# KarypisLab/SLIM

Measured on AMD Instinct MI355X. Metric: item-columns solved/sec (whole node), higher is better.
Workload: dtype f32

## Files before the change

slim_amd/csrc/cd_tile.hpp:

```cpp
#pragma once
#include <type_traits>

#include "cd_wave.hpp"

namespace slimamd {

#ifndef SLIM_TILE_END_ALIGNED
#define SLIM_TILE_END_ALIGNED 1
#endif

constexpr int kTileNW = 16;
constexpr int kTileKMax = 32;
constexpr float kInactive = -__builtin_huge_valf();
__device__ __forceinline__ bool tile_active(float xv) { return xv > -3.0e38f; }

__device__ __forceinline__ void pin(float& v) { asm volatile("" : "+v"(v)); }
__device__ __forceinline__ void pin(int& v) { asm volatile("" : "+v"(v)); }

template <int N>
__device__ __forceinline__ int row_bcast_c(int v) {
  return __builtin_amdgcn_update_dpp(0, v, 0x150 + N, 0xF, 0xF, true);
}
__device__ __forceinline__ int row_bcast(int v, int n) {
  switch (n & 15) {
    case 0: return row_bcast_c<0>(v);
    case 1: return row_bcast_c<1>(v);
    case 2: return row_bcast_c<2>(v);
    case 3: return row_bcast_c<3>(v);
    case 4: return row_bcast_c<4>(v);
    case 5: return row_bcast_c<5>(v);
    case 6: return row_bcast_c<6>(v);
    case 7: return row_bcast_c<7>(v);
    case 8: return row_bcast_c<8>(v);
    case 9: return row_bcast_c<9>(v);
    case 10: return row_bcast_c<10>(v);
    case 11: return row_bcast_c<11>(v);
    case 12: return row_bcast_c<12>(v);
    case 13: return row_bcast_c<13>(v);
    case 14: return row_bcast_c<14>(v);
    default: return row_bcast_c<15>(v);
  }
}
__device__ __forceinline__ float row_bcast(float v, int n) {
  return __int_as_float(row_bcast(__float_as_int(v), n));
}

template <class T>
__device__ __forceinline__ T ld_off(const void* base, const uint32_t byte_off) {
  return *reinterpret_cast<const T*>(reinterpret_cast<const char*>(base) + byte_off);
}

typedef unsigned long long tile_gran_t;

__device__ __forceinline__ void gran_store(tile_gran_t* p, uint32_t epoch, float v) {
  __hip_atomic_store(p, ((tile_gran_t)epoch << 32) | (tile_gran_t)__float_as_uint(v),
                     __ATOMIC_RELAXED, __HIP_MEMORY_SCOPE_AGENT);
}
__device__ __forceinline__ tile_gran_t gran_load(const tile_gran_t* p) {
  return __hip_atomic_load(p, __ATOMIC_RELAXED, __HIP_MEMORY_SCOPE_AGENT);
}

__device__ __forceinline__ int tile_block_id(const SolveArgs& S) {
  const int b = (int)blockIdx.x, g = (int)gridDim.x;
  return S.xcd_swizzle ? (b & 7) * (g >> 3) + (b >> 3) : b;
}

struct GramStore {
  float* G;
  int64_t G_ld;
  const int32_t* gram_pos;
  const float* atypart;
  int64_t x_stride;
  int32_t gram_part16, gram_accum, gram_store;
};
template <int P, int NW>
__device__ __noinline__ void gram_store_lines(const GramStore S, const int* s_item, const int cid, const int mk,
                                              const int K_, const int base, const int ncols, const int wave,
                                              const int lane) {
  const int K = uni(K_);
  float* const G = reinterpret_cast<float*>(uni(reinterpret_cast<int64_t>(S.G)));
  const int64_t G_ld = uni(S.G_ld), x_stride = uni(S.x_stride);
  const float* const part0 =
      reinterpret_cast<const float*>(uni(reinterpret_cast<int64_t>(S.atypart))) + (int64_t)uni(cid) * K * x_stride;
  const bool p16 = uni(S.gram_part16) != 0, accum = uni(S.gram_accum) != 0, mirror = uni(S.gram_store) == 1;
  const int nblk = (uni(ncols) + 63) >> 6;
  const int per = (nblk + K - 1) / K;
  const int bend = (uni(mk) + 1) * per < nblk ? (uni(mk) + 1) * per : nblk;
  for (int blk = uni(mk) * per + uni(wave); blk < bend; blk += NW) {
    const int i = blk * 64 + lane;
    const int pi = i < ncols ? S.gram_pos[i] : -1;
    const bool keep = pi >= base;
    if (__ballot(keep) == 0ull) continue;
    if (!keep) continue;
    for (int h = 0; h < P / 8; ++h) {
      float a[8];
      if (p16) {
        uint32_t n[8];
#pragma unroll
        for (int e = 0; e < 8; ++e) n[e] = 0u;
        const uint4* src = reinterpret_cast<const uint4*>(reinterpret_cast<const uint16_t*>(part0) + (int64_t)i * P) + h;
#pragma unroll 4
        for (int k = 0; k < K; ++k) {
          const uint4 v = *src;
          src = reinterpret_cast<const uint4*>(reinterpret_cast<const float*>(src) + x_stride);
          n[0] += v.x & 0xFFFFu;
          n[1] += v.x >> 16;
          n[2] += v.y & 0xFFFFu;
          n[3] += v.y >> 16;
          n[4] += v.z & 0xFFFFu;
          n[5] += v.z >> 16;
          n[6] += v.w & 0xFFFFu;
          n[7] += v.w >> 16;
        }
#pragma unroll
        for (int e = 0; e < 8; ++e) a[e] = (float)n[e];
      } else {
#pragma unroll
        for (int e = 0; e < 8; ++e) a[e] = 0.0f;
        const float4* src = reinterpret_cast<const float4*>(part0 + (int64_t)i * P) + 2 * h;
#pragma unroll 2
        for (int k = 0; k < K; ++k) {
          const float4 v = src[0], w = src[1];
          src = reinterpret_cast<const float4*>(reinterpret_cast<const float*>(src) + x_stride);
          a[0] += v.x;
          a[1] += v.y;
          a[2] += v.z;
          a[3] += v.w;
          a[4] += w.x;
          a[5] += w.y;
          a[6] += w.z;
          a[7] += w.w;
        }
      }
      int it[8];
#pragma unroll
      for (int e = 0; e < 8; ++e) it[e] = uni(s_item[8 * h + e]);
      if (accum) {
#pragma unroll
        for (int e = 0; e < 8; ++e)
          if (it[e] >= 0) a[e] += G[(int64_t)it[e] * G_ld + i];
      }
#pragma unroll
      for (int e = 0; e < 8; ++e) {
        if (it[e] >= 0) {
          G[(int64_t)it[e] * G_ld + i] = a[e];
// ... 473 lines not shown
          sim = S.simtype == 0 ? a / cn_i : (S.simtype == 1 ? a / ((cn_i + s_cn[qq]) - a) : a);
        }
        x[idx] = sim;
      }
      auto keyof = [](const float f) -> uint32_t {
        const uint32_t b = __float_as_uint(f);
        return (b & 0x80000000u) ? ~b : (b | 0x80000000u);
      };
      const uint32_t key_ninf = keyof(kInactive);
      for (int pass = 0; pass < 4; ++pass) {
        const int shift = 24 - 8 * pass;
        for (int k = tid; k < P * 256; k += NT) hist[k] = 0u;
        __syncthreads();
        for (int64_t idx = tid; idx < n; idx += NT) {
          const int qq = (int)(idx & (P - 1));
          const uint32_t key = keyof(x[idx]);
          if (key == key_ninf) continue;
          const uint32_t hi_mask = pass == 0 ? 0u : (0xFFFFFFFFu << (shift + 8));
          if ((key & hi_mask) == s_prefix[qq]) atomicAdd(&hist[qq * 256 + ((key >> shift) & 255u)], 1u);
        }
        __syncthreads();
        if (tid < P) {
          uint32_t want = s_want[tid], d = 255u;
          for (;; --d) {
            const uint32_t c = hist[tid * 256 + d];
            if (c >= want || d == 0u) break;
            want -= c;
          }
          s_prefix[tid] |= d << shift;
          s_want[tid] = want;
        }
        __syncthreads();
      }
#pragma unroll
      for (int pp = 0; pp < PPW; ++pp) {
        const int pq = wave + pp * NW;
        const uint32_t T = s_prefix[pq];
        int quota = (int)s_want[pq], na = 0;
        for (int ib = 0; ib < ncols; ib += 64) {
          const int i = ib + lane;
          const uint32_t key = i < ncols ? keyof(x[(int64_t)i * P + pq]) : key_ninf;
          const bool cand = key != key_ninf;
          const bool tie = cand && key == T;
          const uint64_t mt = __ballot(tie);
          const bool act = cand && (key > T || (tie && __popcll(mt & lane_lt) < quota));
          quota -= __popcll(mt) < quota ? __popcll(mt) : quota;
          if (i < ncols) x[(int64_t)i * P + pq] = act ? 0.0f : kInactive;
          na += __popcll(__ballot(act));
        }
        if (lane == 0) s_na[pq] = na;
      }
    } else if (S.gram_mode == 3 && S.gram_store != 0) {
      const GramStore gs{S.G, S.G_ld, S.gram_pos, S.atypart, S.x_stride, S.gram_part16, S.gram_accum, S.gram_store};
      gram_store_lines<P, NW>(gs, s_item, cid, mk, K, base, ncols, wave, lane);
    } else if (S.gram_mode == 3) {
      const int64_t n = (int64_t)ncols * P;
      const int64_t per = (n + K - 1) / K;
      const int64_t hi = (mk + 1) * per < n ? (mk + 1) * per : n;
      for (int64_t idx = mk * per + tid; idx < hi; idx += NT) {
        const int i = (int)(idx >> LOGP), qq = (int)(idx & (P - 1));
        const int it = s_item[qq];
        const int pi = S.gram_pos[i];
        if (pi >= base && it >= 0) {
          float a = 0.0f;
          if (S.gram_part16) {
            uint32_t n = 0u;
            for (int k = 0; k < K; ++k)
              n += reinterpret_cast<const uint16_t*>(S.atypart + (int64_t)(cid * K + k) * S.x_stride)[idx];
            a = (float)n;
          } else {
            for (int k = 0; k < K; ++k) a += S.atypart[(int64_t)(cid * K + k) * S.x_stride + idx];
          }
          if (S.gram_accum) a += S.G[(int64_t)it * S.G_ld + i];
          S.G[(int64_t)it * S.G_ld + i] = a;
          if (pi >= base + P) S.G[(int64_t)i * S.G_ld + it] = a;
        }
      }
    } else {
      const int64_t n = (int64_t)ncols * P;
      for (int64_t idx = tid; idx < n; idx += NT) {
        const int i = (int)(idx >> LOGP), qq = (int)(idx & (P - 1));
        const int it = s_item[qq];
        float a = 0.0f;
        if (cached) {
          a = gram_t[idx];
        } else {
          for (int k = 0; k < K; ++k)
            a += S.atypart[(int64_t)(cid * K + k) * S.x_stride + idx];
          if (gram_t != nullptr && mk == 0) gram_t[idx] = a;
        }
        const bool act = it >= 0 && i != it && a > l1;
        x[idx] = act ? 0.0f : kInactive;
        if (act) atomicAdd(&s_na[qq], 1);
      }
    }
    __syncthreads();
    if (S.gram_mode == 3) continue;

    const bool warm = FOLD != 0 && S.icolptr != nullptr && !FSLIM;
    if (warm) {
#pragma unroll
      for (int pp = 0; pp < PPW; ++pp) {
        const int pq = wave + pp * NW;
        const int witem = s_item[pq];
        if (witem >= 0 && witem < S.incols) {
          const int64_t ws = uni(S.icolptr[witem]), we = uni(S.icolptr[witem + 1]);
          for (int64_t e = ws + lane; e < we; e += 64) {
// ... 592 lines not shown
```

slim_amd/csrc/cd_wave.hpp:

```cpp
#pragma once
#include <hip/hip_runtime.h>

#include <cstdint>

#include "cd_perm.hpp"

namespace slimamd {

struct DevMatrix {
  int32_t nrows, ncols;
  int64_t nnz;
  const int64_t* rowptr;
  const int32_t* rowind;
  const float* rowval;
  const int64_t* colptr;
  const int32_t* colind;
  const float* colval;
  const float* cnorm;
  const float* csq;
};

struct SolveArgs {
  float l1, l2, opt_tol;
  int32_t maxniters;
  uint32_t seed;
  int32_t nnbrs;
  int32_t simtype;
  const int32_t* order;
  int32_t nwork;
  int32_t* queue;
  const int64_t* icolptr;
  const int32_t* icolind;
  const float* icolval;
  int32_t incols;
  float* slab;
  int64_t slab_stride;
  int32_t nrows_pad, ncols_pad;
  float* xslab;
  int64_t x_stride;
  int32_t* ulist;
  int64_t u_stride;
  int32_t ngroups;
  uint64_t* trace;
  int32_t cluster;
  const int32_t* ubounds;
  const int64_t* csplit;
  unsigned long long* mailbox;
  float* atypart;
  int32_t exact_gram;
  int32_t bm_shift, bm_words;
  int32_t nheavy;
  int32_t cluster_hi;
  const int32_t* ubounds_hi;
  const int64_t* csplit_hi;
  unsigned long long* mailbox_hi;
  int32_t* queue_hi;
  int64_t nnz_last;
  int32_t hi_prefetch;
  int32_t shard_count, shard_index;
  int32_t xcd_swizzle;
  float* gram;
  int32_t gram_mode;
  float* G;
  int64_t G_ld;
  int32_t* tile_nunion;
  const int32_t* gram_pos;
  int32_t gram_bits;
  int32_t gram_split_stride;
  int32_t gram_accum;
  const uint4* gview;
  const int64_t* gview_base;
  const uint16_t* gview_cnt;
  int32_t gview_ngroups;
  int32_t gview_range0;
  int32_t gview_sentinel;
  int32_t gram_part16;
  int32_t gram_store;
  float* g_save;
  const float* g_load;
  int64_t g_stride;
  int32_t* out_cnt;
  int64_t* out_off;
  int32_t* out_ind;
  float* out_val;
  unsigned long long* out_cursor;
  int64_t out_cap;
  int32_t* overflow;
  int32_t* st_na;
  int32_t* st_sweeps;
  int32_t* st_conv;
  int64_t* st_G;
  int64_t* st_D;
  int64_t* st_U;
  int64_t* st_B;
  float* st_err;
  float* st_obj;
};

constexpr float kEps = 1e-7f;


__device__ __forceinline__ float cd_num(float g, float xeff, float sq) {
  float p = xeff * sq;
  asm volatile("" : "+v"(p));
  return g + p;
}
__device__ __forceinline__ float cd_den(float cn, float l2) { return fmaf(cn, cn, l2); }
__device__ __forceinline__ int uni(int v) { return __builtin_amdgcn_readfirstlane(v); }
__device__ __forceinline__ uint32_t uni(uint32_t v) {
  return (uint32_t)__builtin_amdgcn_readfirstlane((int)v);
}
__device__ __forceinline__ float uni(float v) {
  return __int_as_float(__builtin_amdgcn_readfirstlane(__float_as_int(v)));
}
__device__ __forceinline__ int64_t uni(int64_t v) {
  uint32_t lo = uni((uint32_t)v), hi = uni((uint32_t)((uint64_t)v >> 32));
  return (int64_t)(((uint64_t)hi << 32) | lo);
}
__device__ __forceinline__ int lane_bcast(int v, int src) {
  return __builtin_amdgcn_readlane(v, src);
}
__device__ __forceinline__ float lane_bcast(float v, int src) {
  return __int_as_float(__builtin_amdgcn_readlane(__float_as_int(v), src));
}
__device__ __forceinline__ int64_t lane_bcast(int64_t v, int src) {
  uint32_t lo = (uint32_t)__builtin_amdgcn_readlane((int)(uint32_t)v, src);
  uint32_t hi = (uint32_t)__builtin_amdgcn_readlane((int)(uint32_t)((uint64_t)v >> 32), src);
  return (int64_t)(((uint64_t)hi << 32) | lo);
}

// ... 341 lines not shown
```

slim_amd/csrc/engine.hip:

```cpp
#include <hip/hip_runtime.h>

#include <algorithm>
#include <atomic>
#include <chrono>
#include <cmath>
#include <cstdio>
#include <cstdlib>
#include <cstring>
#include <functional>
#include <mutex>
#include <new>
#include <numeric>
#include <memory>
#include <string>
#include <thread>

#include <rocprim/device/device_radix_sort.hpp>

#include "tile_inst.hpp"
#include "gram_inst.hpp"
#include "gramr_inst.hpp"
#include "gram_sym.hpp"
#include "fslim_gram_inst.hpp"
#include "cd_wave.hpp"
// ... 995 lines not shown
    std::iota(w.order.begin(), w.order.end(), cb);
  }
  if (opt.shard_index < 0 || opt.shard_index >= opt.shard_count)
    throw Refusal{SLIM_ERROR_INPUT, "SLIMGPU_Learn: shard index outside [0, shard count)"};
  std::vector<int32_t>& order = w.order;
  std::stable_sort(order.begin(), order.end(),
                   [&](int32_t a, int32_t b) { return m->h_cost[a] > m->h_cost[b]; });
  if (opt.shard_count > 1) {
    std::vector<int32_t> mine;
    for (int32_t t = 0; t < (int32_t)order.size(); ++t)
      if ((t / 32) % opt.shard_count == opt.shard_index) mine.push_back(order[(size_t)t]);
    order.swap(mine);
  }
  if (opt.build_G && opt.G_rows_end >= 0) {
    auto in_block = [&](int32_t c) { return c >= opt.G_rows_begin && c < opt.G_rows_end; };
    std::stable_partition(order.begin(), order.end(), in_block);
    w.G_block = (int32_t)std::count_if(order.begin(), order.end(), in_block);
  }
  return w;
}

int32_t build_gram(slimgpu_matrix* m, LearnOptions bo, bool zero_first, double* alloc_ms = nullptr) {
  if (zero_first) {
    const double t0 = now_ms();
    const int64_t G_ld = gram_ld(m->ncols);
    drop_screen_cache(m);
    float* dG = m->ws_G.reserve((size_t)m->ncols * (size_t)G_ld);
    if (alloc_ms) *alloc_ms = now_ms() - t0;
    HIP_TRY(hipMemsetAsync(dG, 0, sizeof(float) * (size_t)m->ncols * (size_t)G_ld, m->stream));
    m->G_ld = G_ld;
  }
  if (bo.G_rows_end >= 0 && bo.G_rows_begin == bo.G_rows_end) return SLIM_OK;
  bo.kernel = SLIMGPU_KERNEL_TILE;
  bo.build_G = true;
  bo.heavy_tiles = 0;
  int32_t st = SLIM_OK;
  if (slim_csr_t* none = learn_cd(m, bo, nullptr, &st, nullptr, 0, false)) csr_free(none);
  return st;
}

struct Path {
  int kernel = 0;
  bool use_gram = false, use_gramr = false, use_tile = false, use_lds = false;
  int nrows_pad = 0, ncols_pad = 0;
  size_t vec_floats = 0, lds_need = 0;
  int gram_nw = 0, gram_v = 0;
  GramrFn fn_r = nullptr;
  int gramr_kr = 0, gramr_kl = 0;
  size_t gram_lds = 0;
  KernelFn fn = nullptr;
  int tileP = 32, tileNW = 16;
  int req_cluster = 0;
  size_t gram_bits_lds = 0;
  int gram_passes = 1;
  int wg_slots = 0;
  int nwaves = 1;
  int trace_level = 0;
  bool has_imodel = false;
  bool exact_gram = false;
  bool use_fgram = false, f_block = false;
  int f_stride = 0, f_ustride = 0, f_tab_n = 0, f_waves = 1;
  size_t f_wave_lds = 0, f_union_lds = 0;
  FslimFn fn_f = nullptr;
};

Path choose_kernel(slimgpu_matrix* m, const LearnOptions& opt, int32_t nwork) {
  const int32_t ncols = m->ncols;
  Path p;
  p.nrows_pad = round_up(std::max(m->nrows, 1), 64);
  p.ncols_pad = round_up(ncols, 64);
  p.vec_floats = (size_t)p.nrows_pad + 2 * (size_t)p.ncols_pad;
  p.lds_need = p.vec_floats * sizeof(float);
  p.kernel = opt.kernel;
  const bool gram_fits =
      gram_geometry(p.ncols_pad, &p.gram_nw, &p.gram_v) && opt.nnbrs == 0 && !opt.build_G && ncols > 0;
  const size_t G_bytes = sizeof(float) * (size_t)ncols * (size_t)gram_ld(ncols);
  if (p.kernel == SLIMGPU_KERNEL_GRAM_FSLIM) {
    if (opt.nnbrs <= 0 || opt.build_G)
      throw Refusal{SLIM_ERROR_INPUT, "SLIMGPU_Learn: the item-space FSLIM kernel needs nnbrs > 0"};
    if (m->nonpositive)
      throw Refusal{SLIM_ERROR_INPUT, "SLIMGPU_Learn: the item-space FSLIM kernel needs ratings > 0: with a rating <= 0 "
                                      "a co-rating sum can cancel to 0 and G cannot mark the column as co-rated "
                                      "(the tile kernel solves such matrices)"};
    if (std::min(opt.nnbrs, ncols - 1) > kFslimMaxNbrs)
      throw Refusal{SLIM_ERROR_INPUT, "SLIMGPU_Learn: the item-space FSLIM kernel holds at most 4096 neighbours per "
                                      "problem in LDS (min(nnbrs, ncols - 1) is larger)"};
    if (m->G_ready && m->Gf_dropped) {
      m->G_ready = false;
      m->Gf_dropped = false;
    }
    size_t free_b = 0, total_b = 0;
    HIP_TRY(hipMemGetInfo(&free_b, &total_b));
    if (!m->G_ready && G_bytes + (size_t(4) << 30) > free_b + m->ws_gram.bytes())
      throw Refusal{SLIM_ERROR_MEMORY, "SLIMGPU_Learn: G = R^T R (4 ncols^2 bytes) does not fit the free HBM"};
    p.use_fgram = true;
    return p;
  }
  if (p.kernel == SLIMGPU_KERNEL_GRAM) {
    if (!gram_fits) throw Refusal{SLIM_ERROR_INPUT, "SLIMGPU_Learn: the item-space kernel has no FSLIM form"};
    size_t free_b = 0, total_b = 0;
    HIP_TRY(hipMemGetInfo(&free_b, &total_b));
    if (!m->G_ready && G_bytes + (size_t(4) << 30) > free_b + m->ws_gram.bytes())
      throw Refusal{SLIM_ERROR_MEMORY, "SLIMGPU_Learn: G = R^T R (4 ncols^2 bytes) does not fit the free HBM"};
    p.use_gram = true;
  } else if (p.kernel == SLIMGPU_KERNEL_AUTO && gram_fits && p.lds_need > 64 * 1024 &&
             !std::getenv("SLIM_GPU_NO_GRAMCD")) {
// ... 182 lines not shown
    const char* form = "colfold";
    bool profiled = false;
    if (p.tileP == 32 && opt.nnbrs > 0) {
      p.fn = tile_kernel_p32_fslim(val, nw16);
      form = "fslim";
    } else if (p.tileP == 32 && !prof && !p.has_imodel) {
      p.fn = tile_kernel_p32_cold(val, nw16);
      form = "cold";
    } else if (p.tileP == 32 && !prof && row_fold) {
      p.fn = tile_kernel_p32_rowfold(val, nw16);
      form = "rowfold";
    } else if (p.tileP == 32) {
      p.fn = nw16 ? tile_kernel_p32_nw16(val, prof) : tile_kernel_p32_nw8(val, prof);
      profiled = prof;
    } else {
      p.fn = nw16 ? tile_kernel_p16_nw16(val, prof) : tile_kernel_p16_nw8(val, prof);
      profiled = prof;
    }
    if (p.trace_level >= 1)
      std::fprintf(stderr, "[trace] tile kernel: P %d, %d wavefronts, form %s, %s%s\n", p.tileP, nw16 ? 16 : 8,
                   form, val ? "valued" : "binary", profiled ? ", profiled" : "");
  }
  int waves_per_cu;
  if (p.use_gram) {
    int per_cu = 0;
    const void* kfn = p.use_gramr ? reinterpret_cast<const void*>(p.fn_r) : reinterpret_cast<const void*>(p.fn);
    HIP_TRY(hipFuncSetAttribute(kfn, hipFuncAttributeMaxDynamicSharedMemorySize, (int)p.gram_lds));
    HIP_TRY(hipOccupancyMaxActiveBlocksPerMultiprocessor(&per_cu, kfn, 64 * p.gram_nw, p.gram_lds));
    if (per_cu < 1)
      throw Refusal{SLIM_ERROR, "SLIMGPU_Learn: the item-space kernel does not fit a compute unit of this device"};
    waves_per_cu = per_cu;
  } else if (p.use_lds) {
    waves_per_cu = (int)std::min<size_t>(16, (160 * 1024) / std::max<size_t>(p.lds_need, 1));
    if (waves_per_cu < 1) waves_per_cu = 1;
    if (p.lds_need > 64 * 1024)
      HIP_TRY(hipFuncSetAttribute(reinterpret_cast<const void*>(p.fn),
                                  hipFuncAttributeMaxDynamicSharedMemorySize, (int)p.lds_need));
  } else {
    waves_per_cu = 8;
  }
  p.nwaves = std::max(1, std::min(nwork, m->num_cus * waves_per_cu));
  if (!p.use_gram && !p.use_tile && p.trace_level >= 1)
    std::fprintf(stderr, "[trace] wave kernel: %s, %s, sums %s, %d wavefronts, %zu bytes of LDS\n",
                 p.use_lds ? "lds" : "hbm", m->binary ? "binary" : "valued", p.exact_gram ? "ordered" : "atomic",
                 p.nwaves, p.use_lds ? p.lds_need : (size_t)0);
  p.wg_slots = m->num_cus * (16 / p.tileNW);
  if (p.use_tile) {
    int per_cu = 0;
    const size_t worst_lds = std::max<size_t>(kBitmapBytes, p.gram_bits_lds);
    HIP_TRY(hipFuncSetAttribute(reinterpret_cast<const void*>(p.fn),
                                hipFuncAttributeMaxDynamicSharedMemorySize, (int)worst_lds));
    HIP_TRY(hipOccupancyMaxActiveBlocksPerMultiprocessor(&per_cu, reinterpret_cast<const void*>(p.fn),
                                                         64 * p.tileNW, worst_lds));
    if (per_cu < 1)
      throw Refusal{SLIM_ERROR, "SLIMGPU_Learn: the tile kernel does not fit a compute unit of this device"};
    p.wg_slots = m->num_cus * std::min(per_cu, 16 / p.tileNW);
  }
}

struct TileGeom {
  bool force_k1 = false;
  int clusterK = 1, cluster_lg = 0, nclusters = 0;
  int clusterHi = 0, hi_lg = 0, nheavy = 0, nclusters_hi = 0;
  size_t tile_r = 0, tile_x = 0, tile_u = 0;
  int nwaves = 0;
};

TileGeom plan_tiles(slimgpu_matrix* m, const LearnOptions& opt, const Path& p,
                    const std::vector<int32_t>& order, bool force_k1) {
  const int32_t ncols = m->ncols, nwork = (int32_t)order.size();
  const int tileP = p.tileP;
  TileGeom t;
  t.force_k1 = force_k1;
  int auto_heavy = 0;
  const int ngroups_all = (nwork + tileP - 1) / tileP;
  const int req = p.req_cluster;
  if (force_k1) {
    t.clusterK = 1;
  } else if (req == 1 || req == 2 || req == 4 || req == 8 || req == 16 || req == 32) {
    t.clusterK = req;
  } else {
    int cap = 1;
    while (cap < 16 && (m->nnz / std::max(ncols, 1)) / (2 * cap) >= 512) cap *= 2;
    if (opt.heavy_tiles < 0 && p.tileNW == 16 && ngroups_all >= 16) {
      auto tile_cost = [&](int gI) {
        int64_t c = 0;
        for (int k = gI * tileP; k < std::min((gI + 1) * tileP, nwork); ++k) c += m->h_cost[order[(size_t)k]];
        return c;
      };
      const int64_t med = tile_cost(ngroups_all / 2);
      while (auto_heavy < ngroups_all / 16 && tile_cost(auto_heavy) >= 12 * med) ++auto_heavy;
    }
    const int64_t fill = auto_heavy > 0 ? 4 : 8;
    while (t.clusterK < cap && (int64_t)ngroups_all * t.clusterK < fill * (int64_t)p.wg_slots) t.clusterK *= 2;
  }
  while (t.clusterK > 1 && p.wg_slots / t.clusterK < 1) t.clusterK /= 2;
  for (t.cluster_lg = 0; (1 << t.cluster_lg) < t.clusterK; ++t.cluster_lg) {}
  ensure_cluster_split(m, t.cluster_lg);
  t.tile_r = (size_t)(round_up(m->split[t.cluster_lg].max_rows, 64) + 64) * tileP;
  if (opt.build_G && p.gram_bits_lds && t.clusterK == 32 && !force_k1) t.tile_r = (size_t)64 * tileP;
  t.tile_x = (size_t)p.ncols_pad * tileP;
  t.tile_u = (size_t)p.ncols_pad;
  t.nclusters = std::max(1, std::min(ngroups_all, p.wg_slots / t.clusterK));
  t.nheavy = std::min(opt.heavy_tiles < 0 ? auto_heavy : opt.heavy_tiles, ngroups_all);
  t.clusterHi = opt.heavy_cluster;
  if (const char* e = std::getenv("SLIM_GPU_HEAVY")) {
    int a = 0, b = 0;
    if (std::sscanf(e, "%d,%d", &a, &b) == 2) {
      t.nheavy = std::min(std::max(a, 0), ngroups_all);
      t.clusterHi = b;
    }
  }
  if (t.clusterHi != 2 && t.clusterHi != 4 && t.clusterHi != 8 && t.clusterHi != 16 && t.clusterHi != 32)
    t.clusterHi = std::max(16, std::min(4 * t.clusterK, kTileKMax));
  if (t.clusterHi <= t.clusterK || t.nclusters * t.clusterK < t.clusterHi || force_k1) t.nheavy = 0;
  if (t.nheavy > 0) {
    for (t.hi_lg = 0; (1 << t.hi_lg) < t.clusterHi; ++t.hi_lg) {}
    ensure_cluster_split(m, t.hi_lg);
    t.nclusters_hi = t.nclusters * t.clusterK / t.clusterHi;
    t.tile_r = std::max(t.tile_r, (size_t)(round_up(m->split[t.hi_lg].max_rows, 64) + 64) * tileP);
  }
  size_t free_b = 0, total_b = 0;
  HIP_TRY(hipMemGetInfo(&free_b, &total_b));
  const size_t per_cl = ((t.tile_r + 2 * t.tile_x) * sizeof(float) + t.tile_u * sizeof(int32_t)) * t.clusterK;
  const size_t have = free_b + m->ws_slab.bytes() + m->ws_xslab.bytes() + m->ws_ulist.bytes() +
                      m->ws_part.bytes() + m->ws_gram.bytes();
  const size_t budget = have > (size_t(6) << 30) ? have - (size_t(6) << 30) : have / 2;
  if ((size_t)t.nclusters * per_cl > budget) {
    t.nclusters = (int)std::max<size_t>(1, budget / per_cl);
    t.nclusters_hi = t.nclusters * t.clusterK / std::max(t.clusterHi, 1);
    if (t.nclusters_hi < 1) t.nheavy = 0;
  }
  t.nwaves = t.nclusters * t.clusterK;
  return t;
}

size_t mailbox_stride(int tileP) { return 2 * (size_t)kTileKMax * (size_t)tileP + 8; }

struct Slabs {
  float *slab = nullptr, *xslab = nullptr, *part = nullptr;
  int32_t *ulist = nullptr, *nunion = nullptr;
  unsigned long long* mailbox = nullptr;
  size_t mailbox_words = 0;
  int bm_shift = 0, bm_words = 1;
  size_t tile_lds = 0;
  int32_t *f_n = nullptr, *f_id = nullptr, *f_slot = nullptr;
  float* f_aty = nullptr;
  int f_slice_tiles = 0;
};

Slabs alloc_slabs(slimgpu_matrix* m, const LearnOptions& opt, const Path& p, const TileGeom& t, int32_t nwork,
                  int nwaves) {
  Slabs s;
  const auto evict = evict_cache(m);
  if (p.use_fgram) {
    const size_t ngroups0 = std::max<size_t>(1, ((size_t)nwork + 31) / 32);
    const size_t per_tile = (size_t)32 * (size_t)p.f_stride * 12;
    size_t free_b = 0, total_b = 0;
    HIP_TRY(hipMemGetInfo(&free_b, &total_b));
    const size_t have = free_b + m->ws_fid.bytes() + m->ws_faty.bytes() + m->ws_fslot.bytes();
    size_t tiles = ngroups0;
    if (tiles * per_tile > have / 4) tiles = std::max<size_t>(1, have / 4 / per_tile);
    if (const char* e = std::getenv("SLIM_GPU_FSLIM_SLICE_TILES"); e && std::atoi(e) > 0)
      tiles = std::min<size_t>(tiles, (size_t)std::atoi(e));
    s.f_slice_tiles = (int)tiles;
    const size_t npos = std::min<size_t>((size_t)std::max(nwork, 1), tiles * 32);
    s.f_n = m->ws_fn.reserve(npos, evict);
    s.f_id = m->ws_fid.reserve(npos * (size_t)p.f_stride, evict);
    s.f_aty = m->ws_faty.reserve(npos * (size_t)p.f_stride, evict);
    s.f_slot = m->ws_fslot.reserve(npos * (size_t)p.f_stride, evict);
    s.ulist = m->ws_ulist.reserve((size_t)p.f_ustride * tiles, evict);
    s.nunion = m->ws_nunion.reserve(tiles, evict);
  } else if (p.use_gram) {
    const size_t ngroups0 = ((size_t)nwork + 31) / 32;
    s.xslab = m->ws_xslab.reserve((size_t)p.ncols_pad * (size_t)nwaves, evict);
    if (p.gram_v == 0) s.slab = m->ws_slab.reserve((size_t)p.ncols_pad * (size_t)nwaves, evict);
    s.ulist = m->ws_ulist.reserve((size_t)p.ncols_pad * ngroups0, evict);
    s.nunion = m->ws_nunion.reserve(ngroups0, evict);
  } else if (p.use_tile) {
    s.mailbox_words = (size_t)(std::max(t.nclusters, 1) + t.nclusters_hi) * mailbox_stride(p.tileP);
    s.slab = m->ws_slab.reserve(t.tile_r * (size_t)nwaves, evict);
    s.xslab = m->ws_xslab.reserve(t.tile_x * (size_t)nwaves, evict);
    s.ulist = m->ws_ulist.reserve(t.tile_u * (size_t)nwaves, evict);
    s.mailbox = m->ws_mailbox.reserve(s.mailbox_words, evict);
    s.part = m->ws_part.reserve(t.tile_x * (size_t)nwaves, evict);
    const int64_t range = (int64_t)(t.tile_r / (size_t)p.tileP);
    auto words_at = [&](int sh) { return ((range >> sh) + 1 + 31) / 32; };
    while (words_at(s.bm_shift) * 4 > kBitmapBytes) ++s.bm_shift;
    s.bm_words = (int)words_at(s.bm_shift);
    if (opt.nnbrs > 0) s.bm_words = std::max(s.bm_words, p.tileP * 256);
    s.tile_lds = sizeof(uint32_t) * (size_t)s.bm_words;
    if (p.gram_bits_lds && t.clusterK == 32 && !t.force_k1) {
      s.bm_shift = 0;
      s.bm_words = (int)(p.gram_bits_lds / sizeof(uint32_t));
      s.tile_lds = p.gram_bits_lds;
    }
  } else if (!p.use_lds) {
    s.slab = m->ws_slab.reserve(p.vec_floats * (size_t)nwaves);
  }
  return s;
}

struct ArenaSeg {
  const int32_t* ind;
  const float* val;
  int64_t n;
  DeviceBuffer<int32_t> own_i;
  DeviceBuffer<float> own_v;
};

struct Launch {
  Path p;
  TileGeom t;
  Slabs s;
  int nwaves = 1;
  int32_t *order = nullptr, *cnt = nullptr, *sti = nullptr, *misc = nullptr;
  int64_t *off = nullptr, *stl = nullptr;
  float* stf = nullptr;
  const int64_t* icolptr = nullptr;
  const int32_t* icolind = nullptr;
  const float* icolval = nullptr;
  int32_t incols = 0;
  int gram_mode = 0;
  float* gram = nullptr;
  int gram_geom[6] = {0, 0, 0, 0, 0, 0};
  int gram_pass = 0;
  DeviceBuffer<float> carry;
  int64_t carry_stride = 0;
  bool carry_from_warm = false;
  bool cluster_fallback = false;
  int64_t arena_cap = 0;
  int32_t G_block = 0;
  bool gview_tried = false;
  const uint4* gview = nullptr;
  const int64_t* gview_base = nullptr;
  const uint16_t* gview_cnt = nullptr;
  int32_t gview_ngroups = 0, gview_sentinel = 0;
  size_t gview_bytes = 0;
  double gview_ms = 0;
  const char* gview_why = "";
};

void prepare_launch(slimgpu_matrix* m, const LearnOptions& opt, const std::vector<int32_t>& order,
                    const slim_csr_t* imodel, const slimgpu_model* warm_dev, bool resident, bool all_columns,
                    Launch& L) {
  const int32_t ncols = m->ncols, nwork = (int32_t)order.size();
  const Path& p = L.p;
  hipStream_t stream = m->stream;
  L.nwaves = p.nwaves;
// ... 87 lines not shown
  const TileGeom& t = L.t;
  const int32_t ncols = m->ncols, npend = (int32_t)pending.size();
  hipStream_t stream = m->stream;
  SolveArgs S;
  S.l1 = (float)opt.l1r;
  S.l2 = (float)opt.l2r;
  S.opt_tol = (float)opt.optTol;
  S.maxniters = opt.maxniters;
  S.seed = opt.seed;
  S.nnbrs = opt.nnbrs;
  S.simtype = opt.simtype;
  S.order = L.order;
  S.nwork = npend;
  S.queue = L.misc;
  S.icolptr = L.icolptr;
  S.icolind = L.icolind;
  S.icolval = L.icolval;
  S.incols = L.incols;
  S.slab = L.s.slab;
  S.slab_stride = p.use_tile ? (int64_t)t.tile_r : (int64_t)p.vec_floats;
  S.nrows_pad = p.nrows_pad;
  S.ncols_pad = p.ncols_pad;
  S.xslab = L.s.xslab;
  S.x_stride = (int64_t)t.tile_x;
  S.ulist = L.s.ulist;
  S.u_stride = (int64_t)t.tile_u;
  S.ngroups = (npend + p.tileP - 1) / p.tileP;
  if (opt.build_G && opt.G_rows_end >= 0) S.ngroups = (L.G_block + p.tileP - 1) / p.tileP;
  S.cluster = t.clusterK;
  S.ubounds = p.use_tile ? m->split[t.cluster_lg].ubounds.get() : nullptr;
  S.csplit = p.use_tile ? m->split[t.cluster_lg].csplit.get() : nullptr;
  S.mailbox = L.s.mailbox;
  S.exact_gram = p.exact_gram ? 1 : 0;
  S.atypart = L.s.part;
  S.bm_shift = L.s.bm_shift;
  S.bm_words = L.s.bm_words;
  S.nheavy = p.use_tile ? t.nheavy : 0;
  S.cluster_hi = t.clusterHi;
  S.ubounds_hi = t.nheavy > 0 ? m->split[t.hi_lg].ubounds.get() : nullptr;
  S.csplit_hi = t.nheavy > 0 ? m->split[t.hi_lg].csplit.get() : nullptr;
  S.mailbox_hi = L.s.mailbox ? L.s.mailbox + (size_t)std::max(t.nclusters, 1) * mailbox_stride(p.tileP) : nullptr;
  S.queue_hi = L.misc + 4;
  S.hi_prefetch = 1;
  S.shard_count = opt.shard_count;
  S.shard_index = opt.shard_index;
  S.nnz_last = m->nnz > 0 ? m->nnz - 1 : 0;
  S.xcd_swizzle = 0;
  S.gram_mode = (attempt == 0 && !L.cluster_fallback) ? L.gram_mode : 0;
  S.gram = L.gram;
  S.G = m->ws_G.get();
  S.G_ld = m->G_ld;
  S.tile_nunion = L.s.nunion;
  S.gram_pos = nullptr;
  S.gram_bits = (p.gram_bits_lds && t.clusterK == 32 && L.s.tile_lds == p.gram_bits_lds) ? 2 : 0;
  if (const char* e = std::getenv("SLIM_GPU_GBITS"); e && S.gram_bits) S.gram_bits = std::atoi(e) == 1 ? 1 : 2;
  S.gram_split_stride = t.clusterK + 1;
  S.gram_accum = 0;
  S.gram_store = 0;
  S.gview = nullptr;
  S.gview_base = nullptr;
  S.gview_cnt = nullptr;
  S.gview_ngroups = 0;
  S.gview_range0 = 0;
  S.gview_sentinel = 0;
  S.gram_part16 = S.gram_bits == 2 ? 1 : 0;
  if (const char* e = std::getenv("SLIM_GPU_GPART16"); e && std::atoi(e) == 0) S.gram_part16 = 0;
  S.g_save = nullptr;
  S.g_load = nullptr;
  S.g_stride = 0;
  if (L.carry.get()) {
    S.g_save = L.carry.get();
    S.g_stride = L.carry_stride;
    S.g_load = (L.carry_from_warm && attempt == 0) ? L.carry.get() : nullptr;
  }
  if (L.p.gram_passes > 1) {
    if (S.gram_bits) {
      S.ubounds = m->gsplit.ubounds.get() + 32 * L.gram_pass;
      S.csplit = m->gsplit.csplit.get() + 32 * L.gram_pass;
      S.gram_split_stride = 32 * L.p.gram_passes + 1;
      S.gram_accum = L.gram_pass > 0;
    } else {
      L.p.gram_passes = 1;
      L.gram_pass = 0;
    }
  }
  if (opt.build_G) {
    if (npend != ncols)
      throw Refusal{SLIM_ERROR, "SLIMGPU_Learn: internal: G = R^T R must be built over all columns at once"};
    std::vector<int32_t> pos((size_t)ncols, 0);
    for (int32_t k = 0; k < npend; ++k) pos[(size_t)pending[(size_t)k]] = k;
    int32_t* d_pos = m->ws_nunion.reserve((size_t)ncols, evict_cache(m));
    HIP_TRY(hipMemcpyAsync(d_pos, pos.data(), sizeof(int32_t) * (size_t)ncols, hipMemcpyHostToDevice, stream));
    HIP_TRY(hipStreamSynchronize(stream));
    S.gram_pos = d_pos;
    S.gram_mode = 3;
    S.gram_store = opt.G_rows_end >= 0 ? 1 : 2;
    if (const char* e = std::getenv("SLIM_GPU_GLINES"); e && std::atoi(e) >= 0 && std::atoi(e) < S.gram_store)
      S.gram_store = std::atoi(e);
  }
  if (p.use_gram) {
    S.slab_stride = (int64_t)p.ncols_pad;
    S.x_stride = (int64_t)p.ncols_pad;
    S.u_stride = (int64_t)p.ncols_pad;
    S.ngroups = (npend + 31) / 32;
  }
  if (p.use_fgram) {
    S.u_stride = (int64_t)p.f_ustride;
    S.ngroups = (npend + 31) / 32;
  }
  if (const char* e = std::getenv("SLIM_GPU_HI_PREFETCH")) S.hi_prefetch = std::atoi(e);
  if (p.use_tile)
    HIP_TRY(hipMemsetAsync(L.s.mailbox, 0, sizeof(unsigned long long) * L.s.mailbox_words, stream));
  S.trace = nullptr;
  if (p.use_tile && p.trace_level >= 1) {
    S.trace = m->ws_trace.reserve(16 * (size_t)S.ngroups);
    HIP_TRY(hipMemsetAsync(S.trace, 0, sizeof(uint64_t) * 16 * (size_t)S.ngroups, stream));
  }
  S.out_cnt = L.cnt;
  S.out_off = L.off;
  S.out_ind = d_ai;
  S.out_val = d_av;
  S.out_cursor = reinterpret_cast<unsigned long long*>(L.misc + 2);
  S.out_cap = L.arena_cap;
  S.overflow = L.misc + 1;
  S.st_na = L.sti;
  S.st_sweeps = L.sti + ncols;
  S.st_conv = L.sti + 2 * (size_t)ncols;
  S.st_G = L.stl;
  S.st_D = L.stl + ncols;
  S.st_U = L.stl + 2 * (size_t)ncols;
  S.st_B = L.stl + 3 * (size_t)ncols;
  S.st_err = L.stf;
  S.st_obj = L.stf + ncols;
  return S;
}

void build_gview(slimgpu_matrix* m, Launch& L, const SolveArgs& S, const int32_t* d_colind) {
  L.gview_tried = true;
  if (const char* e = std::getenv("SLIM_GPU_GVIEW"); e && std::atoi(e) == 0) {
    L.gview_why = " (SLIM_GPU_GVIEW=0)";
    return;
  }
  hipStream_t stream = m->stream;
  const double t0 = now_ms();
  const int nranges = 32 * L.p.gram_passes;
  const int ngroups = (S.nwork + 63) / 64;
  const int sentinel = S.bm_words - 64;
  if ((int64_t)nranges * ngroups >= (int64_t(1) << 31) || sentinel >= 65536 || sentinel < 0) {
    L.gview_why = " (ranges beyond 16-bit ids)";
    return;
  }
// ... 141 lines not shown
    P.rank_of = m->ws_rankof.get();
    P.item_of = m->ws_itemof.get();
    P.nchunks = m->Gp_nchunks;
  }

  struct DropView {
    slimgpu_matrix* m;
    ~DropView() {
      m->ws_gview.reset();
      m->ws_gvbase.reset();
      m->ws_gvrows.reset();
      m->ws_gvcnt.reset();
    }
  } drop_view{m};

  Entries E;
  E.cnt.assign((size_t)ncols, 0);
  E.off.assign((size_t)ncols, 0);
  std::vector<int32_t> h_cnt((size_t)ncols, 0);
  std::vector<int64_t> h_off((size_t)ncols, 0);
  std::vector<int32_t> pending = order;
  for (int attempt = 0; attempt < 8 && !pending.empty(); ++attempt) {
    const int32_t npend = (int32_t)pending.size();
    int32_t* d_ai = m->ws_arena_i.reserve((size_t)L.arena_cap, evict_cache(m));
    float* d_av = m->ws_arena_v.reserve((size_t)L.arena_cap, evict_cache(m));
    if (L.gram_mode != 0 && m->ws_gram.get() != L.gram) {
      L.gram_mode = 0;
      L.gram = nullptr;
    }
    HIP_TRY(hipMemcpyAsync(L.order, pending.data(), sizeof(int32_t) * (size_t)npend, hipMemcpyHostToDevice, stream));
    HIP_TRY(hipMemsetAsync(L.misc, 0, sizeof(int32_t) * 16, stream));
    if (attempt > 0) L.t.nheavy = 0;
    SolveArgs S = solve_args(m, opt, L, pending, attempt, d_ai, d_av);
    const int clusterK = L.t.clusterK;
    if (opt.build_G && S.gram_bits == 2 && !L.gview_tried) build_gview(m, L, S, A.colind);
    if (opt.build_G && S.gram_bits == 2 && L.gview) {
      S.gview = L.gview;
      S.gview_base = L.gview_base;
      S.gview_cnt = L.gview_cnt;
      S.gview_ngroups = L.gview_ngroups;
      S.gview_range0 = 32 * L.gram_pass;
      S.gview_sentinel = L.gview_sentinel;
    }
    if (opt.build_G && p.trace_level >= 1) {
      const bool in_passes = S.gram_bits != 0 && p.gram_passes > 1;
      std::fprintf(stderr, "[trace] G builder: form %s, clusters of %d, pass %d of %d, %d users at most per member\n",
                   S.gram_bits == 2 ? "bits2" : (S.gram_bits == 1 ? "bits1" : "lines"), clusterK, L.gram_pass + 1,
                   p.gram_passes, in_passes ? m->gsplit.max_rows : m->split[L.t.cluster_lg].max_rows);
      if (S.gview)
        std::fprintf(stderr, "[trace] G builder: ids from view, %zu bytes = %.3f x 2 bytes per nnz, built in %.1f ms\n",
                     L.gview_bytes, (double)L.gview_bytes / (2.0 * (double)std::max<int64_t>(m->nnz, 1)), L.gview_ms);
      else
        std::fprintf(stderr, "[trace] G builder: ids from csc%s\n", S.gram_bits == 2 ? L.gview_why : "");
    }

    const int launch_waves = p.use_tile ? std::max(1, std::min((npend + p.tileP - 1) / p.tileP, L.t.nclusters)) * clusterK
                                        : std::max(1, std::min(npend, L.nwaves));
    HIP_TRY(hipEventRecord(ev0, stream));
    if (p.use_gramr)
      hipLaunchKernelGGL(gramr_union_fn(), dim3(S.ngroups), dim3(gramr_union_threads()), 0, stream, A, S, P);
    else if (p.use_gram)
      hipLaunchKernelGGL(gram_union_fn(), dim3(S.ngroups), dim3(64), 0, stream, A, S);
    if (S.nheavy > 0 && launch_waves < L.t.clusterHi) S.nheavy = 0;
    int launch_now = launch_waves;
    if (p.use_tile && clusterK > 1 && !L.cluster_fallback && test_hook("SLIM_GPU_TEST_DROP_MEMBER")) {
      launch_now -= 1;
      S.nheavy = 0;
    }
    const int nxcd = m->num_cus % 32 == 0 ? m->num_cus / 32 : 1;
    if (p.use_tile && clusterK > 1 && nxcd == 8 && launch_now % 8 == 0 &&
        (launch_now / 8) % clusterK == 0 && (S.nheavy == 0 || (launch_now / 8) % L.t.clusterHi == 0)) {
      S.xcd_swizzle = 1;
      if (const char* e = std::getenv("SLIM_GPU_XCD")) S.xcd_swizzle = std::atoi(e) != 0;
    }
    if (p.use_fgram) {
      FslimArgs F{};
      F.stride = p.f_stride;
      F.nbr_n = L.s.f_n;
      F.nbr_id = L.s.f_id;
      F.nbr_aty = L.s.f_aty;
      F.nbr_slot = L.s.f_slot;
      F.wave_lds = (int32_t)p.f_wave_lds;
      F.tab_n = p.f_tab_n;
      const int slice = L.s.f_slice_tiles * 32;
      for (int pos0 = 0; pos0 < npend; pos0 += slice) {
        F.pos0 = pos0;
        F.npos = std::min(slice, npend - pos0);
        if (pos0 > 0) HIP_TRY(hipMemsetAsync(L.misc, 0, sizeof(int32_t), stream));
        hipLaunchKernelGGL(fslim_select_fn(), dim3(F.npos), dim3(kFslimSelectThreads), 0, stream, A, S, F);
        hipLaunchKernelGGL(fslim_union_fn(), dim3((F.npos + 31) / 32), dim3(kFslimUnionThreads), p.f_union_lds, stream,
                           A, S, F);
        hipLaunchKernelGGL(p.fn_f, dim3(std::max(1, std::min((F.npos + p.f_waves - 1) / p.f_waves, L.nwaves))),
                           dim3(64 * p.f_waves), p.f_wave_lds * (size_t)p.f_waves, stream, A, S, F);
        HIP_TRY(hipGetLastError());
      }
    } else if (p.use_gramr)
      hipLaunchKernelGGL(p.fn_r, dim3(launch_now), dim3(kGramrNT), p.gram_lds, stream, A, S, P);
    else
      hipLaunchKernelGGL(p.fn, dim3(launch_now), dim3(p.use_gram ? 64 * p.gram_nw : (p.use_tile ? 64 * p.tileNW : 64)),
                         p.use_gram ? p.gram_lds : (p.use_lds ? p.lds_need : (p.use_tile ? L.s.tile_lds : 0)),
                         stream, A, S);
    HIP_TRY(hipGetLastError());
    HIP_TRY(hipEventRecord(ev1, stream));

    int32_t h_misc[4];
    HIP_TRY(hipMemcpyAsync(h_misc, L.misc, sizeof(h_misc), hipMemcpyDeviceToHost, stream));
// ... 687 lines not shown
```

Measured before the change: 2141.

## Stage partial Gram sums through per-wave LDS tiles for coalesced single reads

In the Gram line-store path with 32-item tiles, each wave now reads the K partial sums for a 64-column block once, using contiguous 16-byte loads laid out to match memory. It transposes them through a padded per-wave LDS staging tile, then writes G rows with lane-per-column stores. Previously each lane strided through its own row in 4 rounds, which gave poorly coalesced loads. The host sizes dynamic LDS to hold the staging tiles and may raise the kernel's LDS request, which can lower occupancy. The host falls back when the tiles do not fit or when SLIM_GPU_GREAD=0.

```diff
diff --git a/slim_amd/csrc/cd_tile.hpp b/slim_amd/csrc/cd_tile.hpp
--- a/slim_amd/csrc/cd_tile.hpp
+++ b/slim_amd/csrc/cd_tile.hpp
@@ -73,10 +73,19 @@
   int64_t x_stride;
   int32_t gram_part16, gram_accum, gram_store;
 };
+constexpr int kGramStageLd = 66;
+constexpr int kGramStageBytes = 32 * kGramStageLd * (int)sizeof(float);
+typedef __attribute__((address_space(3))) float lds_float_t;
+typedef __attribute__((address_space(3))) const int lds_cint_t;
+__device__ __forceinline__ void wave_lds_sync() {
+  __builtin_amdgcn_fence(__ATOMIC_RELEASE, "wavefront");
+  __builtin_amdgcn_wave_barrier();
+  __builtin_amdgcn_fence(__ATOMIC_ACQUIRE, "wavefront");
+}
 template <int P, int NW>
-__device__ __noinline__ void gram_store_lines(const GramStore S, const int* s_item, const int cid, const int mk,
-                                              const int K_, const int base, const int ncols, const int wave,
-                                              const int lane) {
+__device__ __noinline__ void gram_store_lines(const GramStore S, lds_cint_t* const s_item, lds_float_t* const stage,
+                                              const int cid, const int mk, const int K_, const int base,
+                                              const int ncols, const int wave, const int lane) {
   const int K = uni(K_);
   float* const G = reinterpret_cast<float*>(uni(reinterpret_cast<int64_t>(S.G)));
   const int64_t G_ld = uni(S.G_ld), x_stride = uni(S.x_stride);
@@ -90,7 +99,97 @@
     const int i = blk * 64 + lane;
     const int pi = i < ncols ? S.gram_pos[i] : -1;
     const bool keep = pi >= base;
-    if (__ballot(keep) == 0ull) continue;
+    const uint64_t km = __ballot(keep);
+    if (km == 0ull) continue;
+    if (P == 32 && stage != nullptr) {
+      const char* const run0 = reinterpret_cast<const char*>(part0) + (int64_t)blk * (p16 ? 64 * P * 2 : 64 * P * 4);
+      const int64_t mstride = x_stride * (int64_t)sizeof(float);
+#pragma unroll 1
+      for (int r = 0; r < 4; ++r) {
+        if (p16) {
+          uint32_t n[8];
+#pragma unroll
+          for (int e = 0; e < 8; ++e) n[e] = 0u;
+          const int c = 16 * r + (lane >> 2);
+          if ((km >> c) & 1ull) {
+            const char* src = run0 + (r * 1024 + lane * 16);
+#pragma unroll 4
+            for (int k = 0; k < K; ++k) {
+              const uint4 v = *reinterpret_cast<const uint4*>(src);
+              src += mstride;
+              n[0] += v.x & 0xFFFFu;
+              n[1] += v.x >> 16;
+              n[2] += v.y & 0xFFFFu;
+              n[3] += v.y >> 16;
+              n[4] += v.z & 0xFFFFu;
+              n[5] += v.z >> 16;
+              n[6] += v.w & 0xFFFFu;
+              n[7] += v.w >> 16;
+            }
+          }
+          lds_float_t* const out = stage + (8 * (lane & 3)) * kGramStageLd + c;
+#pragma unroll
+          for (int e = 0; e < 8; ++e) out[e * kGramStageLd] = (float)n[e];
+        } else {
+          float a[8];
+#pragma unroll
+          for (int e = 0; e < 8; ++e) a[e] = 0.0f;
+          const int c = 16 * r + (lane >> 3);
+          const bool lo = (km >> c) & 1ull, hi = (km >> (c + 8)) & 1ull;
+          if (lo || hi) {
+            const char* src = run0 + (r * 2048 + lane * 16);
+#pragma unroll 2
+            for (int k = 0; k < K; ++k) {
+              float4 v = make_float4(0.f, 0.f, 0.f, 0.f), w = v;
+              if (lo) v = *reinterpret_cast<const float4*>(src);
+              if (hi) w = *reinterpret_cast<const float4*>(src + 1024);
+              src += mstride;
+              a[0] += v.x;
+              a[1] += v.y;
+              a[2] += v.z;
+              a[3] += v.w;
+              a[4] += w.x;
+              a[5] += w.y;
+              a[6] += w.z;
+              a[7] += w.w;
+            }
+          }
+          lds_float_t* const out = stage + (4 * (lane & 7)) * kGramStageLd + c;
+#pragma unroll
+          for (int e = 0; e < 4; ++e) {
+            out[e * kGramStageLd] = a[e];
+            out[e * kGramStageLd + 8] = a[4 + e];
+          }
+        }
+      }
+      wave_lds_sync();
+#pragma unroll 1
+      for (int h = 0; h < 4; ++h) {
+        float a[8];
+        int it[8];
+#pragma unroll
+        for (int e = 0; e < 8; ++e) {
+          a[e] = stage[(8 * h + e) * kGramStageLd + lane];
+          it[e] = uni(s_item[8 * h + e]);
+        }
+        if (keep) {
+          if (accum) {
+#pragma unroll
+            for (int e = 0; e < 8; ++e)
+              if (it[e] >= 0) a[e] += G[(int64_t)it[e] * G_ld + i];
+          }
+#pragma unroll
+          for (int e = 0; e < 8; ++e) {
+            if (it[e] >= 0) {
+              G[(int64_t)it[e] * G_ld + i] = a[e];
+              if (mirror && pi >= base + P) G[(int64_t)i * G_ld + it[e]] = a[e];
+            }
+          }
+        }
+      }
+      wave_lds_sync();
+      continue;
+    }
     if (!keep) continue;
     for (int h = 0; h < P / 8; ++h) {
       float a[8];
@@ -670,7 +769,9 @@
       }
     } else if (S.gram_mode == 3 && S.gram_store != 0) {
       const GramStore gs{S.G, S.G_ld, S.gram_pos, S.atypart, S.x_stride, S.gram_part16, S.gram_accum, S.gram_store};
-      gram_store_lines<P, NW>(gs, s_item, cid, mk, K, base, ncols, wave, lane);
+      lds_float_t* const stage =
+          S.gram_read ? (lds_float_t*)s_bits + wave * (kGramStageBytes / (int)sizeof(float)) : (lds_float_t*)nullptr;
+      gram_store_lines<P, NW>(gs, (lds_cint_t*)s_item, stage, cid, mk, K, base, ncols, wave, lane);
     } else if (S.gram_mode == 3) {
       const int64_t n = (int64_t)ncols * P;
       const int64_t per = (n + K - 1) / K;
diff --git a/slim_amd/csrc/cd_wave.hpp b/slim_amd/csrc/cd_wave.hpp
--- a/slim_amd/csrc/cd_wave.hpp
+++ b/slim_amd/csrc/cd_wave.hpp
@@ -76,6 +76,7 @@
   int32_t gview_sentinel;
   int32_t gram_part16;
   int32_t gram_store;
+  int32_t gram_read;
   float* g_save;
   const float* g_load;
   int64_t g_stride;
diff --git a/slim_amd/csrc/engine.hip b/slim_amd/csrc/engine.hip
--- a/slim_amd/csrc/engine.hip
+++ b/slim_amd/csrc/engine.hip
@@ -1071,6 +1071,8 @@
   int tileP = 32, tileNW = 16;
   int req_cluster = 0;
   size_t gram_bits_lds = 0;
+  size_t gram_stage_lds = 0;
+  const char* gram_stage_why = "";
   int gram_passes = 1;
   int wg_slots = 0;
   int nwaves = 1;
@@ -1359,6 +1361,33 @@
                                 hipFuncAttributeMaxDynamicSharedMemorySize, (int)worst_lds));
     HIP_TRY(hipOccupancyMaxActiveBlocksPerMultiprocessor(&per_cu, reinterpret_cast<const void*>(p.fn),
                                                          64 * p.tileNW, worst_lds));
+    if (opt.build_G && per_cu >= 1) {
+      const size_t stage = (size_t)kGramStageBytes * (size_t)p.tileNW;
+      const char* e = std::getenv("SLIM_GPU_GREAD");
+      if (e && std::atoi(e) == 0) {
+        p.gram_stage_why = "SLIM_GPU_GREAD=0";
+      } else if (p.tileP != 32) {
+        p.gram_stage_why = "16-item tiles";
+      } else if (stage > worst_lds) {
+        hipFuncAttributes fa{};
+        HIP_TRY(hipFuncGetAttributes(&fa, reinterpret_cast<const void*>(p.fn)));
+        int per_cu_s = 0;
+        if (fa.sharedSizeBytes + stage <= (size_t)160 * 1024) {
+          HIP_TRY(hipFuncSetAttribute(reinterpret_cast<const void*>(p.fn),
+                                      hipFuncAttributeMaxDynamicSharedMemorySize, (int)stage));
+          HIP_TRY(hipOccupancyMaxActiveBlocksPerMultiprocessor(&per_cu_s, reinterpret_cast<const void*>(p.fn),
+                                                               64 * p.tileNW, stage));
+        }
+        if (per_cu_s >= std::min(per_cu, 16 / p.tileNW)) {
+          p.gram_stage_lds = stage;
+          per_cu = per_cu_s;
+        } else {
+          p.gram_stage_why = "no room in LDS";
+        }
+      } else {
+        p.gram_stage_lds = stage;
+      }
+    }
     if (per_cu < 1)
       throw Refusal{SLIM_ERROR, "SLIMGPU_Learn: the tile kernel does not fit a compute unit of this device"};
     p.wg_slots = m->num_cus * std::min(per_cu, 16 / p.tileNW);
@@ -1451,6 +1480,7 @@
   size_t mailbox_words = 0;
   int bm_shift = 0, bm_words = 1;
   size_t tile_lds = 0;
+  bool gram_words = false;
   int32_t *f_n = nullptr, *f_id = nullptr, *f_slot = nullptr;
   float* f_aty = nullptr;
   int f_slice_tiles = 0;
@@ -1501,7 +1531,9 @@
       s.bm_shift = 0;
       s.bm_words = (int)(p.gram_bits_lds / sizeof(uint32_t));
       s.tile_lds = p.gram_bits_lds;
-    }
+      s.gram_words = true;
+    }
+    if (opt.build_G) s.tile_lds = std::max(s.tile_lds, p.gram_stage_lds);
   } else if (!p.use_lds) {
     s.slab = m->ws_slab.reserve(p.vec_floats * (size_t)nwaves);
   }
@@ -1695,11 +1727,12 @@
   S.G_ld = m->G_ld;
   S.tile_nunion = L.s.nunion;
   S.gram_pos = nullptr;
-  S.gram_bits = (p.gram_bits_lds && t.clusterK == 32 && L.s.tile_lds == p.gram_bits_lds) ? 2 : 0;
+  S.gram_bits = (p.gram_bits_lds && t.clusterK == 32 && L.s.gram_words) ? 2 : 0;
   if (const char* e = std::getenv("SLIM_GPU_GBITS"); e && S.gram_bits) S.gram_bits = std::atoi(e) == 1 ? 1 : 2;
   S.gram_split_stride = t.clusterK + 1;
   S.gram_accum = 0;
   S.gram_store = 0;
+  S.gram_read = 0;
   S.gview = nullptr;
   S.gview_base = nullptr;
   S.gview_cnt = nullptr;
@@ -1740,6 +1773,7 @@
     S.gram_store = opt.G_rows_end >= 0 ? 1 : 2;
     if (const char* e = std::getenv("SLIM_GPU_GLINES"); e && std::atoi(e) >= 0 && std::atoi(e) < S.gram_store)
       S.gram_store = std::atoi(e);
+    S.gram_read = (S.gram_store != 0 && p.gram_stage_lds && L.s.tile_lds >= p.gram_stage_lds) ? 1 : 0;
   }
   if (p.use_gram) {
     S.slab_stride = (int64_t)p.ncols_pad;
@@ -1987,6 +2021,11 @@
                      L.gview_bytes, (double)L.gview_bytes / (2.0 * (double)std::max<int64_t>(m->nnz, 1)), L.gview_ms);
       else
         std::fprintf(stderr, "[trace] G builder: ids from csc%s\n", S.gram_bits == 2 ? L.gview_why : "");
+      if (S.gram_read)
+        std::fprintf(stderr, "[trace] G builder: sums read once, %zu of %zu bytes of LDS hold the staging tiles\n",
+                     p.gram_stage_lds, L.s.tile_lds);
+      else if (S.gram_store != 0)
+        std::fprintf(stderr, "[trace] G builder: sums read in rounds (%s)\n", p.gram_stage_why);
     }
 
     const int launch_waves = p.use_tile ? std::max(1, std::min((npend + p.tileP - 1) / p.tileP, L.t.nclusters)) * clusterK
```

Result: faster. 2279 (median of 6 runs) (+6.4%).
